# taki0112/vit-tensorflow

Hardware: AMD Instinct MI355X
Metric: images/sec (fwd+bwd) ViT-B/16 224px bf16 (higher is better)
Workload: dtype bf16; 1 GPU; vit_b16_224 fwd+bwd, batch 256/GPU, N(0,1) NHWC images resident in HBM, random-init weights, softmax-CE cotangent, dropout 0; global_batch=256, parallelism=dp1, compute=bf16

## Files before the change

vit-tensorflow_amd/csrc/env.hip:

```cpp
#include "env.h"

#include <cstdio>
#include <cstdlib>
#include <cstring>
#include <mutex>
#include <set>
#include <string>

namespace {

const VitxEnvSwitch kSwitches[] = {
    {"VITX_GENERIC_GEMM", VITX_ENV_PATH, "1: every Dense on the k-ordered fp32-FMA kernel instead of the MFMA kernels"},
    {"VITX_GENERIC_ATTN", VITX_ENV_PATH, "1: materialised attention (batched products + row softmax) instead of the fused kernel"},
    {"VITX_DEEPVIT_FUSED", VITX_ENV_PATH, "0: DeepViT Re-attention forward as batched GEMMs + head-axis kernels instead of the one-kernel form"},
    {"VITX_DEEPVIT_FUSED_BWD", VITX_ENV_PATH, "0: DeepViT Re-attention backward as batched GEMMs + point / row kernels"},
    {"VITX_CAIT_FUSED", VITX_ENV_PATH, "0: CaiT talking-heads forward as batched GEMMs + chain kernel instead of the one-kernel form"},
    {"VITX_CAIT_QKV_CAT", VITX_ENV_PATH, "0: CaiT patch stage: to_q and to_kv as two Dense launches each way (rounds d(y1) twice)"},
    {"VITX_LN_SCALE_FUSED", VITX_ENV_PATH, "0: CaiT LayerScale VJP as a pass of its own instead of on the LayerNorm VJP (bias gradient from the bf16 rounding)"},
    {"VITX_CHAIN_MFMA", VITX_ENV_PATH, "0: talking-heads chain kernels with in-lane FMAs instead of the fp32 matrix pipe"},
    {"VITX_UNFUSED_HEADOPS", VITX_ENV_PATH, "1: head-axis operations (mix / softmax / LayerNorm over heads) as one kernel each"},
    {"VITX_WGRAD_TRANSPOSE", VITX_ENV_PATH, "1: weight gradients through explicit bf16 transposes + the NT kernel"},
    {"VITX_GELU_TABLE", VITX_ENV_PATH, "0: fc1 epilogue evaluates the degree-7 polynomial GELU instead of the LDS table (another rounding of gelu, both inside a bf16 ulp)"},
    {"VITX_LAST_BLOCK_FULL", VITX_ENV_PATH, "1: the last block of a cls-pooled bf16 ViT on every token row instead of the class rows only (same logits; eight of its parameter gradients sum in another order); read per forward"},
    {"VITX_X3_ATTN", VITX_ENV_PATH, "BF16X3 handles: 1 fused split-operand attention (default), 2 materialised scores + split-operand products, 0 exact fp32 products"},
    {"VITX_F32_MFMA", VITX_ENV_TUNING, "0: parity-mode GEMMs on the scalar-FMA kernel instead of the fp32 matrix pipe (same bits)"},
    {"VITX_GEMM_KERNEL", VITX_ENV_TUNING, "force one NT tile variant (1, 2, 3, 5, 6, 7, 9, 10, 11, 13; +256 direct / +512 LDS-staged epilogue); every variant adds in the same K order"},
    {"VITX_GEMM_TAIL_KERNEL", VITX_ENV_TUNING, "with VITX_GEMM_KERNEL=13 / 11: tile variant (1, 3, 10) of the tail launch (tail balancing)"},
    {"VITX_GEMM_TAIL", VITX_ENV_TUNING, "1: the per-shape measurement also times the tail-balanced forms (off by default: loses inside the step)"},
    {"VITX_GEMM_AUTOTUNE", VITX_ENV_TUNING, "0: static variant rule instead of the first-launch measurement"},
    {"VITX_GEMM_AUTOTUNE_LOG", VITX_ENV_TUNING, "1: print the measured variant choices"},
    {"VITX_GEMM_WALK", VITX_ENV_TUNING, "0: no XCD-owned row bands in the persistent NT kernel"},
    {"VITX_GEMM_GRID", VITX_ENV_TUNING, "n: persistent workgroups per launch (default 256)"},
    {"VITX_GEMM_PHASE", VITX_ENV_TUNING, "n: start-phase offsets between the persistent workgroups of an XCD (sleeps only)"},
    {"VITX_EPI_WIDE", VITX_ENV_TUNING, "0: 4-B instead of 16-B-per-lane epilogue accesses"},
    {"VITX_NT", VITX_ENV_TUNING, "bits: non-temporal stores (1 = gelu' of the fc1 epilogue, 16 = d(y) of the fc1 / qkv input gradients; default 17)"},
    {"VITX_REVERSE", VITX_ENV_TUNING, "bits: row tiles walked back to front for operands larger than the memory-side cache (1 forward, 2 input gradients)"},
    {"VITX_REVERSE_MIN_MB", VITX_ENV_TUNING, "operand size from which VITX_REVERSE applies"},
    {"VITX_MLP_BWD_ORDER", VITX_ENV_TUNING, "0: fc2 weight gradient between the producer and the consumers of d(hpre)"},
    {"VITX_BGEMM_PAIRS", VITX_ENV_TUNING, "0: the batched products of the materialised attention backward as four launches instead of two (same bits)"},
    {"VITX_ATTN_BWD_SPLIT", VITX_ENV_TUNING, "1: fused attention backward as two launches (same bits)"},
    {"VITX_GLP_SKIP", VITX_ENV_TUNING, "0: LayerNorm VJPs always write the bf16 copy of the residual gradient"},
    {"VITX_SCORE_BF16", VITX_ENV_TUNING, "0: DeepViT / CaiT score tensors that only batched products read stay fp32 planes (same bits)"},
    {"VITX_LN_CORESIDENT", VITX_ENV_TUNING, "1: LayerNorm VJP of 768-wide bf16 rows as 4-wave, 96-register blocks that fit beside a resident weight-gradient GEMM (experiment; partials summed in another order)"},
    {"VITX_LN_CO_BLOCKS", VITX_ENV_TUNING, "blocks of the co-resident LayerNorm VJP form (default 1024; 256 = one 4-wave block per CU, what fits beside a resident GEMM workgroup)"},
    {"VITX_SIDE_STREAM", VITX_ENV_TUNING, "0 one stream; 1 weight gradients on a lowest-priority side stream (default); 2 the same at the highest priority"},
    {"VITX_LN_REDUCE_SIDE_ROWS", VITX_ENV_TUNING, "LayerNorm VJPs of fewer rows keep their small reductions on the main stream (default 8192)"},
    {"VITX_SC_KEEP_MB", VITX_ENV_TUNING, "budget of the score tensors kept per block for the backward; blocks beyond it recompute (same bits)"},
    {"VITX_RECOMPUTE_SCORES", VITX_ENV_TUNING, "1: materialised attention recomputes its score tensors in the backward (same bits)"},
    {"VITX_WGRAD_WGS", VITX_ENV_TUNING, "workgroups per weight-gradient launch (default 128 up to 24576 token rows, else 256); changes the split-K slice count: fixed-order sums in another order"},
    {"VITX_SG_BLOCKS", VITX_ENV_TUNING, "blocks per LayerScale-gradient launch"},
    {"VITX_DV_CPI", VITX_ENV_TUNING, "chunks per image of the DeepViT one-kernel forward (tests: the multi-tile loop at small batches)"},
    {"VITX_COMM_PRIORITY", VITX_ENV_TUNING, "priority of the communication stream: 1 highest (default), 0 default, -1 lowest"},
    {"VITX_COMM_TIMING", VITX_ENV_TUNING, "0: no event brackets around the collectives (every Dense launch behind a bucket then takes the one-tile form)"},
    {"VITX_COMM_WAIT_ON_CHAIN", VITX_ENV_TUNING, "1: the compute stream (not the communication stream) waits for the weight-gradient stream's share of a reported range"},
    {"VITX_COMM_STREAM_EARLY", VITX_ENV_TUNING, "0: the communication stream is created at vitx_comm_overlap instead of with the handle's other streams (A/B: it may then share a command-processor pipe with the compute stream)"},
    {"VITX_COMM_SHARED", VITX_ENV_TUNING, "1: the Dense launches behind a bucket take the one-tile-per-workgroup form for as long as its collective was measured to last (default 0: persistent grids throughout, faster with emulated collectives)"},
    {"VITX_RCCL_LIB", VITX_ENV_TUNING, "path of the collective library to dlopen instead of librccl.so (tests/fake_rccl: two ranks on one GPU)"},
    {"VITX_GEMM_STAGGER", VITX_ENV_DIAG, "bits reach the NT kernels' experiment field: 1 no DMA wait, 2 no DMA issue (WRONG GEMM results)"},
    {"VITX_GEMM_XP", VITX_ENV_DIAG, "1: vitx_bench_gemm accepts the NT kernels' experiment bits (results invalid)"},
    {"VITX_TN_XP", VITX_ENV_DIAG, "bits: weight-gradient kernel without DMA wait / DMA issue / fragment reads (WRONG weight gradients)"},
    {"VITX_DV_XP", VITX_ENV_DIAG, "bits: DeepViT one-kernel forward without kept tensors / stage 2 / stage 3 (WRONG results)"},
    {"VITX_DVB_XP", VITX_ENV_DIAG, "bits: DeepViT one-kernel backward without one of its stages (WRONG results)"},
    {"VITX_BENCH_ZERO", VITX_ENV_DIAG, "vitx_bench_gemm on zero operands (DVFS / power-limit experiment)"},
    {"VITX_GEMM_STAMPS", VITX_ENV_DIAG, "vitx_bench_gemm prints the cycle stamps of the tile phases (needs the stamps build of gemm_bf16_pipe.hip)"},
};
constexpr int kNumSwitches = (int)(sizeof(kSwitches) / sizeof(kSwitches[0]));

#ifdef VITX_DIAG
constexpr int kDiagBuild = 1;
#else
constexpr int kDiagBuild = 0;
#endif

}

const VitxEnvSwitch* vitx_env_table(int* n) {
  if (n) *n = kNumSwitches;
  return kSwitches;
}
int vitx_env_diag_build() { return kDiagBuild; }

const char* vitx_env(const char* name) {
  const VitxEnvSwitch* sw = nullptr;
  for (int i = 0; i < kNumSwitches; ++i)
    if (std::strcmp(kSwitches[i].name, name) == 0) { sw = &kSwitches[i]; break; }
  if (!sw) {
    fprintf(stderr, "[vitx] internal error: environment switch %s is not in the registry (csrc/env.hip)\n", name);
    abort();
  }
  const char* v = getenv(name);
  if (v && sw->cls == VITX_ENV_DIAG && !kDiagBuild) {
    static std::mutex mu;
    static std::set<std::string> told;
    std::lock_guard<std::mutex> lk(mu);
    if (told.insert(name).second)
      fprintf(stderr, "[vitx] %s is a diagnostic switch that may corrupt results: ignored by this (release) library; use lib/libvitx_diag.so "
                      "(python vit-tensorflow_amd/build.py --diag)\n", name);
    return nullptr;
  }
  return v;
}
```

vit-tensorflow_amd/csrc/gemm_bf16_tn.hip:

```cpp
#include "gemm_bf16_common.h"

namespace {

__device__ __forceinline__ bf16x8 tr_frag(const char* p0, const char* p1) {
  typedef __attribute__((address_space(3))) s16x4 lds_s16x4;
  const s16x4 lo = __builtin_amdgcn_ds_read_tr16_b64_v4i16((lds_s16x4*)p0);
  const s16x4 hi = __builtin_amdgcn_ds_read_tr16_b64_v4i16((lds_s16x4*)p1);
  union { struct { s16x4 a, b; } s; bf16x8 v; } u;
  u.s.a = lo; u.s.b = hi;
  return u.v;
}

template <int BT, int WM, int WN, int MODE>
__global__ __launch_bounds__(WM * WN * 64) void gemm_bf16_tn_kernel(Bf16GemmArgs g, EpiParams ep, int tiles_m, int tiles_n,
                                                                    int kt_per_split) {
  constexpr int NW = WM * WN;
  constexpr int WTM = BT / WM, WTN = BT / WN;
  constexpr int MT = WTM / 32, NT = WTN / 32;
  constexpr int ROWB = BT * 2;
  constexpr int LPR = ROWB / 16;
  constexpr int RPI = 64 / LPR;
  constexpr int OP_BYTES = BK * ROWB, STAGE = 2 * OP_BYTES;
  constexpr int INSTR = BK / RPI / NW;
  static_assert(BK % (RPI * NW) == 0, "token rows must split evenly over the waves");
  extern __shared__ __attribute__((aligned(16))) char smem[];

  const int nwg = gridDim.x, bid = blockIdx.x;
  const int xcd = bid & 7, q8 = nwg >> 3, r8 = nwg & 7;
  const int work = (xcd < r8 ? xcd * (q8 + 1) : r8 * (q8 + 1) + (xcd - r8) * q8) + (bid >> 3);
  const int tiles = tiles_m * tiles_n;
  const int z = work / tiles;
  const int logical = work - z * tiles;
  const int tile_m = logical / tiles_n, tile_n = logical - tile_m * tiles_n;
  const int nk_total = g.K / BK;
  const int kt0 = z * kt_per_split;
  const int nk = min(kt_per_split, nk_total - kt0);

  const int tid = threadIdx.x, lane = tid & 63;
  const int wave = __builtin_amdgcn_readfirstlane(tid >> 6);
  const int wm = wave / WN, wn = wave - wm * WN;

  const bf16_t* Ag = g.A + (int64_t)kt0 * BK * g.lda + (int64_t)tile_m * BT;
  const bf16_t* Bg = g.B + (int64_t)kt0 * BK * g.ldb + (int64_t)tile_n * BT;
  uint32_t offA[INSTR], offB[INSTR];
#pragma unroll
  for (int i = 0; i < INSTR; ++i) {
    const int row = (wave * INSTR + i) * RPI + lane / LPR;
    const int pc = lane % LPR;
    const int c = ((((pc >> 1) ^ (2 * (row & 3))) << 1) | (pc & 1));
    offA[i] = (uint32_t)(row * (int)g.lda + c * 8) * 2u - (uint32_t)((i & 3) * 1024);
    offB[i] = (uint32_t)(row * (int)g.ldb + c * 8) * 2u - (uint32_t)((i & 3) * 1024);
  }
  constexpr int P = 2 * INSTR;
  constexpr int Q = MT * NT;
  constexpr int N3 = (P + 2) / 3, N0 = (P + 1) / 3, N1 = P - N3 - N0;
  const i32x4 rsA = vitx_make_rsrc(Ag), rsB = vitx_make_rsrc(Bg);
  const uint32_t lds_w = vitx_lds_addr(smem) + (uint32_t)wave * (INSTR * 1024u);
  const uint32_t a_kstep = (uint32_t)(BK * g.lda * 2), b_kstep = (uint32_t)(BK * g.ldb * 2);
  auto issue_piece = [&](int buf, int kt, auto p_c) {
    constexpr int p = decltype(p_c)::value;
    const uint32_t base = lds_w + (uint32_t)buf * STAGE;
    if constexpr (p < INSTR) {
      if constexpr ((p & 3) == 0) vitx_dma16(rsA, base + p * 1024, offA[p], (uint32_t)kt * a_kstep);
      else vitx_dma16_cont<(p & 3) * 1024>(rsA, offA[p], (uint32_t)kt * a_kstep);
    } else {
      constexpr int q = p - INSTR;
      if constexpr ((q & 3) == 0) vitx_dma16(rsB, base + OP_BYTES + q * 1024, offB[q], (uint32_t)kt * b_kstep);
      else vitx_dma16_cont<(q & 3) * 1024>(rsB, offB[q], (uint32_t)kt * b_kstep);
    }
  };
  auto stage = [&](int buf, int kt) { static_for<P>([&](auto p_c) { issue_piece(buf, kt, p_c); }); };

  f32x16 acc[MT][NT];
#pragma unroll
  for (int i = 0; i < MT; ++i)
#pragma unroll
    for (int j = 0; j < NT; ++j)
#pragma unroll
      for (int r = 0; r < 16; ++r) acc[i][j][r] = 0.f;

  const int q = lane & 15, G = lane >> 4, khalf = lane >> 5;
  const int trow = q >> 2;
  const int piece = (G & 1) * 32 + (q & 3) * 8;
  auto row_addr = [&](int m, int feat_byte) {
    const int gran = (feat_byte >> 5) ^ (2 * (m & 3));
    return m * ROWB + (gran << 5) + (feat_byte & 31);
  };
  bf16x8 fa[2][MT], fb[2][NT];
  auto load_frags = [&](bf16x8(&af)[MT], bf16x8(&bfr)[NT], const char* base, int ks) {
    const int m0 = 16 * ks + 8 * khalf + trow, m1 = m0 + 4;
#pragma unroll
    for (int i = 0; i < MT; ++i) {
      const int fbyte = (wm * WTM + i * 32) * 2 + piece;
      af[i] = tr_frag(base + row_addr(m0, fbyte), base + row_addr(m1, fbyte));
    }
#pragma unroll
    for (int j = 0; j < NT; ++j) {
      const int fbyte = (wn * WTN + j * 32) * 2 + piece;
      bfr[j] = tr_frag(base + OP_BYTES + row_addr(m0, fbyte), base + OP_BYTES + row_addr(m1, fbyte));
    }
  };
  auto mfma_range = [&](auto cur_c, auto first_c, auto last_c) {
    constexpr int CUR = decltype(cur_c)::value, FIRST = decltype(first_c)::value, LAST = decltype(last_c)::value;
    static_for<(LAST > FIRST ? LAST - FIRST : 0)>([&](auto d) {
      constexpr int idx = FIRST + decltype(d)::value, i = idx / NT, j = idx % NT;
      acc[i][j] = __builtin_amdgcn_mfma_f32_32x32x16_bf16(fb[CUR][j], fa[CUR][i], acc[i][j], 0, 0, 0);
    });
  };
  const int xp = g.stagger;
  auto handover = [&]() {
    if (xp & 1) asm volatile("s_waitcnt lgkmcnt(0)" ::: "memory");
    else asm volatile("s_waitcnt vmcnt(0) lgkmcnt(0)" ::: "memory");
    __builtin_amdgcn_s_barrier();
    asm volatile("" ::: "memory");
  };

  if (nk > 0) stage(0, 0);
  if (nk > 1) stage(1, 1);
  handover();
  load_frags(fa[0], fb[0], smem, 0);
  bool pending = false;
  constexpr int QH = Q < 2 ? Q : 2;
  for (int kt = 0; kt < nk; ++kt) {
    const char* base = smem + (kt & 1) * STAGE;
    static_for<BK / 16>([&](auto ks_c) {
      constexpr int ks = decltype(ks_c)::value, CUR = ks & 1;
      constexpr int NP = ks == 3 ? N3 : (ks == 0 ? N0 : (ks == 1 ? N1 : 0));
      constexpr int FP = ks == 3 ? 0 : (ks == 0 ? N3 : N3 + N0);
      if constexpr (ks + 1 < BK / 16) {
        mfma_range(ic<CUR>{}, ic<0>{}, ic<QH>{});
        __builtin_amdgcn_sched_barrier(0);
        if (!(xp & 4)) load_frags(fa[CUR ^ 1], fb[CUR ^ 1], base, ks + 1);
      } else {
        handover();
        mfma_range(ic<CUR>{}, ic<0>{}, ic<QH>{});
        __builtin_amdgcn_sched_barrier(0);
        if (!(xp & 4)) load_frags(fa[0], fb[0], smem + ((kt + 1) & 1) * STAGE, 0);
        pending = kt + 2 < nk && !(xp & 2);
      }
      __builtin_amdgcn_sched_barrier(0);
      if constexpr (NP > 0) {
        const int ikt = ks == 3 ? kt + 2 : kt + 1;
        const int ibuf = ikt & 1;
        static_for<NP>([&](auto d_c) {
          constexpr int d = decltype(d_c)::value;
          mfma_range(ic<CUR>{}, ic<(QH + d < Q ? QH + d : Q)>{}, ic<(QH + 1 + d < Q ? QH + 1 + d : Q)>{});
          if (pending) issue_piece(ibuf, ikt, ic<FP + d>{});
          __builtin_amdgcn_sched_barrier(0);
        });
        mfma_range(ic<CUR>{}, ic<(QH + NP < Q ? QH + NP : Q)>{}, ic<Q>{});
        if constexpr (FP + NP == P) pending = false;
      } else {
        mfma_range(ic<CUR>{}, ic<QH>{}, ic<Q>{});
      }
      __builtin_amdgcn_sched_barrier(0);
    });
  }

  const int64_t out_off = (int64_t)z * ep.partial_stride;
  const bool interior = epilogue_fast_ok(ep, MODE) && (tile_m + 1) * BT <= ep.M && (tile_n + 1) * BT <= ep.N;
  const float4 z4 = make_float4(0.f, 0.f, 0.f, 0.f);
#pragma unroll
  for (int i = 0; i < MT; ++i) {
    const int row = tile_m * BT + wm * WTM + i * 32 + (lane & 31);
#pragma unroll
    for (int j = 0; j < NT; ++j) {
      const int col0 = tile_n * BT + wn * WTN + j * 32 + 4 * khalf;
#pragma unroll
      for (int qq = 0; qq < 4; ++qq) {
        const float4 v = make_float4(acc[i][j][4 * qq], acc[i][j][4 * qq + 1], acc[i][j][4 * qq + 2], acc[i][j][4 * qq + 3]);
        if (interior) epilogue_fast4<MODE, bf16_t, false, false>(ep, row, col0 + 8 * qq, v, z4, z4, z4, out_off);
        else epilogue_apply4<MODE, bf16_t>(ep, row, col0 + 8 * qq, v, out_off);
      }
    }
  }
}

template <int BT, int WM, int WN>
void launch_tn_variant(const Bf16GemmArgs& g, const EpiParams& ep, hipStream_t s) {
  constexpr int SMEM = 2 * 2 * BK * BT * 2;
  auto kern = gemm_bf16_tn_kernel<BT, WM, WN, EPI_PARTIAL>;
  vitx_set_max_smem((const void*)kern, SMEM);
  const int tiles_m = (int)ceil_div(g.M, BT), tiles_n = (int)ceil_div(g.N, BT);
  const int nk = g.K / BK;
  const int split = g.split_k > 1 ? g.split_k : 1;
  const int per = (int)ceil_div(nk, split);
  const int zs = (int)ceil_div(nk, per);
  dim3 grid((unsigned)(tiles_m * tiles_n * zs)), block(WM * WN * 64);
  hipLaunchKernelGGL(kern, grid, block, SMEM, s, g, ep, tiles_m, tiles_n, per);
}

}

int gemm_bf16_tn_tile(int kernel, int M, int N) { kernel &= 15; return (kernel == 1 || (M <= 128 && N <= 128)) ? 128 : 256; }
void launch_gemm_bf16_tn(const Bf16GemmArgs& g0, const EpiParams& ep, hipStream_t s) {
  static const int xp = [] {
    const char* v = vitx_env("VITX_TN_XP");
    const int x = v ? atoi(v) : 0;
    if (x) fprintf(stderr, "[vitx] VITX_TN_XP=%d: timing experiment -- weight gradients are WRONG in this process\n", x);
    return x;
  }();
  Bf16GemmArgs g = g0;
  g.stagger = xp;
  {
    const int nk = g.K / BK, split = g.split_k > 1 ? g.split_k : 1;
    const int64_t slice_rows = ceil_div(nk, split) * BK;
    if ((slice_rows * std::max(g.lda, g.ldb) + 256) * 2 >= (1LL << 31)) {
      fprintf(stderr, "[vitx] launch_gemm_bf16_tn: a K slice of %lld rows x %lld features exceeds the 2 GiB buffer range -- NOT launched; use more slices\n",
              (long long)slice_rows, (long long)std::max(g.lda, g.ldb));
      return;
    }
  }
  if (gemm_bf16_tn_tile(g.kernel, g.M, g.N) == 128) launch_tn_variant<128, 2, 2>(g, ep, s);
  else launch_tn_variant<256, 2, 4>(g, ep, s);
}
```

vit-tensorflow_amd/csrc/kernels.h:

```cpp
#pragma once
#include "common.h"
#include "epilogue.h"

struct GenericGemmArgs {
  const void* A = nullptr;
  const void* B = nullptr;
  int M = 0, N = 0, K = 0;
  int64_t sam = 0, sak = 1, sbk = 0, sbn = 1;
  int nb = 1, nh = 1;
  int64_t sAb = 0, sAh = 0, sBb = 0, sBh = 0;
  int k_last = 0;
  int x3 = 0;
};
void launch_gemm_generic(const GenericGemmArgs& g, const EpiParams& ep, int mode, int ta, int tb, int to, hipStream_t s);
bool gemm_f32_mfma_supported(const GenericGemmArgs& g, int ta, int tb, int to);
void launch_gemm_f32_mfma(const GenericGemmArgs& g, const EpiParams& ep, int mode, hipStream_t s);
void gemm_f32_mfma_read_env();
bool gemm_bf16x3_supported(const GenericGemmArgs& g, int ta, int tb, int to);
void launch_gemm_bf16x3(const GenericGemmArgs& g, const EpiParams& ep, int mode, hipStream_t s);

bool headchain_supported(int h, int nk);
int64_t headchain_ws_elems(int h);
void launch_cait_chain_fwd(const float* s0, const float* wpre, const float* wpost, float* a1_or_null, float* a2, int b, int h, int nq, int nk,
                           int64_t ld, hipStream_t s);
void launch_cait_chain_bwd(const float* s0, const float* a1, float* da_inout, const float* wpre, const float* wpost, float* ws, float* dwpre,
                           float* dwpost, int b, int h, int nq, int nk, int64_t ld, hipStream_t s, bf16_t* ds_lp = nullptr);
bool cait_chain_bwd_bf16_out_ok();
void launch_deepvit_chain_fwd(float* s0_inout, const float* wre, const float* gamma, const float* beta, float* mixed_or_null, float* a2, int keep,
                              int b, int h, int nq, int nk, int64_t ld, float eps, hipStream_t s);
void launch_deepvit_chain_bwd(const float* a0, const float* mixed, float* da_inout, const float* wre, const float* gamma, float* ws, float* dwre,
                              float* dgamma, float* dbeta, int b, int h, int nq, int nk, int64_t ld, float eps, hipStream_t s);

bool bgemm_mfma_supported(const GenericGemmArgs& g, int ta, int tb, int to, int mode);
void launch_bgemm_mfma(const GenericGemmArgs& g, const EpiParams& ep, int ta, int to, hipStream_t s);
void launch_bgemm_mfma_pair(const GenericGemmArgs& g1, const EpiParams& ep1, int ta1, int to1, const GenericGemmArgs& g2, const EpiParams& ep2, int ta2,
                            int to2, hipStream_t s);

struct Bf16GemmArgs {
  const bf16_t* A = nullptr;
  const bf16_t* B = nullptr;
  int64_t lda = 0, ldb = 0;
  int M = 0, N = 0, K = 0;
  int split_k = 1;
  int kernel = 0;
  unsigned long long* stamps = nullptr;
  int phase = 0;
  int reverse_m = 0;
  int shared_gpu = 0;
  int walk = 0;
  int stagger = 0;
  int tail = 0;
};
void launch_gemm_bf16(const Bf16GemmArgs& g, const EpiParams& ep, int mode, hipStream_t s);
int gemm_bf16_variant_for(int mode, int M, int N, int K, int has_scale, int shared_gpu);
bool gemm_bf16_gelu_table_active();
int gemm_bf16_tile_m(int kernel, int M, int N);
int gemm_bf16_tile_n(int kernel, int M, int N);
int gemm_bf16_num_slices(int K, int split_k);
void gemm_bf16_set_shared_gpu(int on);
void gemm_bf16_allow_320(int on);
void launch_gemm_bf16_tn(const Bf16GemmArgs& g, const EpiParams& ep, hipStream_t s);
int gemm_bf16_tn_tile(int kernel, int M, int N);

bool attn_bf16_supported(int n, int dim_head);
void launch_attn_bf16_fwd(const bf16_t* qkv, bf16_t* o, float* lse, int b, int n, int h, float scale, const bf16_t* zero_page, int reverse,
                          hipStream_t s, int nq_live = 0);
bool attn_x3_supported(int n, int dim_head);
void launch_attn_x3_fwd(const float* qkv, float* o, float* lse, int b, int n, int h, float scale, hipStream_t s);
void launch_attn_x3_bwd(const float* qkv, const float* o, const float* d_o, const float* lse, float* dqkv, int b, int n, int h, float scale, hipStream_t s);
void launch_attn_bf16_bwd(const bf16_t* qkv, const bf16_t* o, const bf16_t* d_o, const float* lse, float* dsum_ws,
                          bf16_t* dqkv, int b, int n, int h, float scale, const bf16_t* zero_page, hipStream_t s, int nq_live = 0);

constexpr int ATTN_STREAM_MAX_N = 1 << 20;
bool attn_stream_supported(int n, int dim_head);
bool attn_stream_fits(int b, int n, int h);
void launch_attn_stream_fwd(const bf16_t* qkv, bf16_t* o, float* lse, int b, int n, int h, float scale, hipStream_t s);
void launch_attn_stream_bwd(const bf16_t* qkv, const bf16_t* o, const bf16_t* d_o, const float* lse, float* dsum_ws, bf16_t* dqkv, int b, int n, int h,
                            float scale, hipStream_t s);

constexpr int LSA_N_MAX = 288;
bool attn_lsa_supported(int n, int dim_head);
int64_t attn_lsa_ws_elems(int b, int n, int h);
void launch_attn_lsa_fwd(const void* qkv, void* o, float* lse, int is_bf16, int b, int n, int h, int dim_head, const float* temperature, hipStream_t s);
void launch_attn_lsa_bwd(const void* qkv, const void* o, const void* d_o, const float* lse, float* dsum_ws, void* dqkv, int is_bf16, int b, int n, int h,
                         int dim_head, const float* temperature, float* dtemperature, float* part_ws, hipStream_t s);
bool attn_small_supported(int n, int dim_head);
void launch_attn_small_fwd(const void* qkv, void* o, float* lse, int is_bf16, int b, int n, int h, int dim_head, float scale, hipStream_t s,
                           const float* bias = nullptr);
void launch_attn_small_bwd(const void* qkv, const void* o, const void* d_o, const float* lse, float* dsum_ws, void* dqkv, int is_bf16, int b, int n, int h,
                           int dim_head, float scale, hipStream_t s, const float* bias = nullptr);
bool attn_window_supported(int n, int dim_head);
void launch_attn_window_fwd(const bf16_t* qkv, bf16_t* o, float* lse, const float* bias, int b, int n, int h, float scale, hipStream_t s);
void launch_attn_window_bwd(const bf16_t* qkv, const bf16_t* o, const bf16_t* d_o, const float* lse, bf16_t* dqkv, const float* bias, int b, int n, int h,
                            float scale, hipStream_t s);
void launch_cf_to_dilated(const float* x, float* tokens, int b, int H, int W, int g, int c, hipStream_t s);
void launch_cf_from_dilated(const float* tokens, float* x, int b, int H, int W, int g, int c, hipStream_t s);
struct CfDpbParams { const float* t[14]; };
int64_t cf_dpb_ws_elems(int wsz);
void launch_cf_dpb_bias(const CfDpbParams& p, int d4, int wsz, float* ws, float* bias, hipStream_t s);
void launch_cf_cols_put(const float* src, float* dst, int64_t rows, int w, int ld, int col0, hipStream_t s);
void launch_cf_cols_get(const float* src, float* dst, int64_t rows, int w, int ld, int col0, hipStream_t s);

void launch_spt_fwd(const float* img, void* rows, int rows_bf16, int64_t ldo, float* mean, float* rstd, const float* gamma, const float* beta, int b,
                    int H, int W, int C, int p, float eps, hipStream_t s);
int64_t spt_bwd_ws_elems(int feat);
void launch_spt_bwd(const float* img, float* d_rows, int64_t ld, const float* mean, const float* rstd, const float* gamma, float* ws, float* dgamma,
                    float* dbeta, int want_dx, int b, int H, int W, int C, int p, hipStream_t s);
void launch_spt_dimg(const float* dx, int64_t ld, float* dimg, int b, int H, int W, int C, int p, hipStream_t s);

void launch_cct_im2col(const float* x, float* rows, int b, int H, int W, int C, int k, int st, int Kp, hipStream_t s);
void launch_cct_relu_maxpool_fwd(const float* conv, float* out, int b, int H, int W, int C, int k, int st, hipStream_t s);
void launch_cct_relu_maxpool_bwd(const float* conv, const float* dout, float* dconv, int b, int H, int W, int C, int k, int st, hipStream_t s);

void launch_nest_to_blocks(const float* x, const float* pos, float* tokens, int b, int nb, int hb, int wb, int c, hipStream_t s, int nbx = 0);
void launch_nest_from_blocks(const float* tokens, float* x, int b, int nb, int hb, int wb, int c, hipStream_t s, int nbx = 0);
void launch_nest_dpos(const float* dtokens, float* part, float* dpos, int nseq, int n, int c, hipStream_t s);
void launch_nest_maxpool_fwd(const float* x, float* out, int b, int H, int W, int C, int k, int st, hipStream_t s);
void launch_nest_maxpool_bwd(const float* x, const float* dout, float* dx, int b, int H, int W, int C, int k, int st, hipStream_t s);

bool attn_fewkey_supported(int nq, int nk, int dim_head);
void launch_attn_fewkey_fwd(const bf16_t* q, const bf16_t* kv, bf16_t* o, float* lse, int b, int nq, int nk, int heads, int64_t ldq, int64_t ldkv,
                            int64_t ldo, float scale, hipStream_t s);
void launch_attn_fewkey_bwd(const bf16_t* q, const bf16_t* kv, const bf16_t* o, const bf16_t* d_o, const float* lse, bf16_t* dq, bf16_t* dkv, int b, int nq,
                            int nk, int heads, int64_t ldq, int64_t ldkv, int64_t ldo, int64_t lddo, int64_t lddq, int64_t lddkv, float scale, hipStream_t s);

constexpr int MANYKEY_MAX = 320;
bool attn_manykey_supported(int nq, int nk, int dim_head);
void launch_attn_manykey_fwd(const bf16_t* q, const bf16_t* kv, bf16_t* o, float* lse, int b, int nq, int nk, int heads, int64_t ldq, int64_t ldkv,
                             int64_t ldo, float scale, hipStream_t s);
void launch_attn_manykey_bwd(const bf16_t* q, const bf16_t* kv, const bf16_t* o, const bf16_t* d_o, const float* lse, bf16_t* dq, bf16_t* dkv, int b, int nq,
                             int nk, int heads, int64_t ldq, int64_t ldkv, int64_t ldo, int64_t lddo, int64_t lddq, int64_t lddkv, float scale, hipStream_t s);

void launch_twins_patch_gather(const float* x, float* out, int b, int H, int W, int C, int p, int64_t ld, hipStream_t s);
void launch_twins_patch_scatter(const float* dpatches, int64_t ld, float* dx, int b, int H, int W, int C, int p, hipStream_t s);
void launch_twins_kunfold(const void* x, void* out, int is_bf16, int b, int H, int W, int C, int k, int64_t ldo, hipStream_t s);
void launch_twins_kfold_add(const void* dwin, int64_t ld, void* dx, int is_bf16, int b, int H, int W, int C, int k, hipStream_t s);
void launch_twins_peg_fwd(const float* x, const float* kern, const float* bias, float* out, int b, int H, int W, int C, int kp, hipStream_t s);
void launch_twins_peg_bwd_dx(const float* dy, const float* kern, float* dx, int b, int H, int W, int C, int kp, hipStream_t s);
int64_t twins_peg_ws_elems(int C, int kp);
void launch_twins_peg_bwd_dkern(const float* x, const float* dy, float* ws, float* dkern, int b, int H, int W, int C, int kp, hipStream_t s);

int64_t cvt_dwbn_ws_elems(int C, int k);
void launch_cvt_dwbn_fwd(const void* x, int is_bf16, const float* kern, const float* gamma, const float* beta, const float* mov_mean, const float* mov_var,
                         int training, float eps, float* conv, double* stats, void* y, int64_t ldy, float* ws, int b, int H, int W, int C, int k, int st,
                         hipStream_t s);
void launch_cvt_bn_bwd(const void* dy, int is_bf16, int64_t lddy, const float* conv, const double* stats, const float* gamma, float* dgamma, float* dbeta,
                       float* dconv, float* ws, int64_t rows, int C, hipStream_t s);
void launch_cvt_dw_bwd_dkern(const void* x, int is_bf16, const float* dconv, float* ws, float* dkern, int b, int H, int W, int C, int k, int st, hipStream_t s);
void launch_cvt_dw_bwd_dx(const float* dconv_q, const float* kern_q, const float* dconv_kv, const float* kern_kv, int st_kv, void* dx, int is_bf16, int b, int H,
                          int W, int C, int k, hipStream_t s);

void launch_unfold(const float* img, void* out, int out_bf16, int b, int H, int W, int C, int ph, int pw,
                   int64_t ldo, hipStream_t s);
void launch_fold_add(const float* dpatches, int64_t ld, float* dimg, int b, int H, int W, int C, int ph, int pw, hipStream_t s);
void extract_patches_geometry(int H, int W, int k, int st, int* oh, int* ow, int* pad_top, int* pad_left);
void launch_extract_patches(const float* x, float* out, int b, int H, int W, int C, int k, int st, hipStream_t s);
void launch_extract_patches_bwd(const float* dout, float* dx, int b, int H, int W, int C, int k, int st, hipStream_t s);
void launch_cls_pos_row(float* x, const float* cls, const float* pos, int b, int ntok, int d, int64_t ldx, hipStream_t s);
void launch_layernorm_fwd(const float* x, int64_t ldx, const float* gamma, const float* beta, void* y, int y_bf16,
                          int64_t ldy, float* mean, float* rstd, int rows, int d, float eps, hipStream_t s);
void launch_layernorm_bwd(const void* dy, int dy_bf16, int64_t lddy, const float* x, int64_t ldx, const float* mean,
                          const float* rstd, const float* gamma, const float* g_in, int64_t ldgi, float* g_out, int64_t ldgo,
                          void* g_lp, int64_t ldglp, float* partial_ws, float* dgamma, float* dbeta, float* gsum, int rows, int d,
                          hipStream_t s, int* deferred = nullptr);
void launch_layernorm_bwd_reduce(float* partial_ws, int nparts, int d, float* dgamma, float* dbeta, float* gsum, hipStream_t s);
int64_t layernorm_bwd_ws_elems(int d);
bool layernorm_bwd_scale_ok(int d);
void launch_layernorm_bwd_scale(const bf16_t* dy, int64_t lddy, const float* x, int64_t ldx, const float* mean, const float* rstd, const float* gamma,
                                const float* g_in, int64_t ldgi, float* g_out, int64_t ldgo, bf16_t* dbr, int64_t lddbr, const bf16_t* nf, int64_t ldnf,
                                const float* nscale, float* partial_ws, int rows, int d, hipStream_t s, int* nparts);
void launch_layernorm_bwd_scale_reduce(float* partial_ws, int nparts, int d, float* dgamma, float* dbeta, float* dscale, float* dbias, const float* nscale,
                                       hipStream_t s);
void launch_colsum(const void* x, int is_bf16, int64_t ld, int rows, int cols, float* partial_ws, float* out, hipStream_t s);
int64_t colsum_ws_elems(int cols);
void launch_reduce_partials(const float* partial, int nparts, int64_t stride, int64_t n, float* out, float alpha, hipStream_t s);
void launch_reduce_partials3(const float* partial, int nparts, int64_t stride, int64_t seg, int nseg, float* out0, float* out1, float* out2,
                             float* ws2, float alpha, hipStream_t s);
void launch_convert_weight(const float* w, int in, int out, bf16_t* wn, int64_t ldwn, bf16_t* wt, int64_t ldwt, hipStream_t s);
struct ConvertDesc { const float* w; bf16_t* wn; bf16_t* wt; int64_t ldwn, ldwt; int in, out, tiles_x, block0; };
void launch_convert_weights_batched(const ConvertDesc* descs_dev, int n, int total_blocks, hipStream_t s);
void launch_transpose_bf16(const bf16_t* in, int64_t ldi, int rows, int cols, bf16_t* out, int64_t ldo, hipStream_t s);
void launch_convert(const float* in, int64_t ldi, void* out, int out_bf16, int64_t ldo, int rows, int cols, int64_t out_cols_zero_to,
                    hipStream_t s);
void launch_to_f32(const void* in, int in_bf16, int64_t ldi, float* out, int64_t ldo, int rows, int cols, hipStream_t s);
void launch_set_token_row(float* x, const float* tok, int b, int ntok, int row, int d, hipStream_t s);
void launch_copy_rows(const void* src, int64_t src_stride_bytes, void* dst, int64_t dst_stride_bytes, int rows, int row_bytes, hipStream_t s);
void launch_mean_pool(const float* x, int b, int ntok, int d, float* out, hipStream_t s, int stride_tok = 0);
void launch_mean_pool_bwd(const float* dp, int b, int ntok, int d, float* g, hipStream_t s, int stride_tok = 0);
void launch_batch_reduce(const float* g, int b, int ntok, int d, int j0, int nj, float* out, hipStream_t s);
void launch_extract_rows(const float* g, int b, int ntok, int tok_off, int np, int d, void* out, int out_bf16, int64_t ldo, hipStream_t s);
void launch_sum_rows(const float* in, int rows, int d, float* out, hipStream_t s);
void launch_ce_grad(const float* logits, int64_t ld, const int32_t* labels, int b, int nc, float inv_batch, float* dlogits,
                    float* loss, hipStream_t s);
void launch_adamw(float* p, const float* g, float* m, float* v, int64_t n, float lr, float b1, float b2, float eps, float wd, int step, hipStream_t s);
void launch_sgd(float* p, const float* g, float* m, int64_t n, float lr, float mom, float wd, hipStream_t s);
void launch_fill_zero(void* p, int64_t bytes, hipStream_t s);
void launch_fill_random_bf16(bf16_t* p, int64_t n, uint32_t seed, float scale, hipStream_t s);
void launch_max_rel_diff(const void* a, const void* b, int is_bf16, int64_t rows, int cols, int64_t lda, int64_t ldb, float* out_max, hipStream_t s);
void launch_dropout(void* x, int is_bf16, int64_t n, float rate, uint64_t seed, uint32_t site, hipStream_t s);
void launch_axpy_resid(const float* resid, const float* f, const float* scale, float* out, void* keep, int keep_bf16, int64_t rows, int d,
                       hipStream_t s);
void launch_branch_grad(const float* g, const float* scale, void* out, int out_bf16, int64_t rows, int d, float rate, uint64_t seed,
                        uint32_t site, hipStream_t s);
void launch_resid_add(const float* resid, const void* t, int t_bf16, float* out, int64_t n, hipStream_t s);

void launch_softmax_rows(float* sc, int64_t rows, int n, int64_t ld, hipStream_t s);
void launch_softmax_bwd_rows(const float* p, float* dp_inout, int64_t rows, int n, int64_t ld, hipStream_t s);
int64_t deepvit_point_bwd_ws_elems(int h);
void launch_deepvit_point_bwd(const float* a0, float* da_inout, const float* w, const float* gamma, float* ws, float* dw,
                              float* dgamma, float* dbeta, int b, int h, int nq, int nk, int64_t ld, float eps, hipStream_t s);
bool deepvit_attn_fused_supported(int h, int dim_head, int nq, int nk);
bool cait_attn_fused_supported(int h, int dim_head, int nq, int nk);
void launch_cait_attn_fwd(const bf16_t* q, const bf16_t* k, const bf16_t* v, int64_t ldq, int64_t ldk, int64_t ldv, int64_t qb, int64_t kb, int64_t vb,
                          bf16_t* o, int64_t ldo, int64_t ob, const float* wpre, const float* wpost, float* s0_keep, float* a1_keep, float* a2_keep,
                          int keep, int b, int h, int nq, int nk, int64_t ld, float scale, const bf16_t* zero_page, hipStream_t s);
int64_t deepvit_attn_bwd_ws_elems(int b, int h, int nq);
void launch_deepvit_attn_bwd(const bf16_t* q, const bf16_t* k, const bf16_t* v, int64_t ldq, int64_t ldk, int64_t ldv, int64_t qb, int64_t kb, int64_t vb,
                             const bf16_t* d_o, int64_t ldo, int64_t ob, const float* p_keep, const float* w, const float* gamma, float* ds_out,
                             bf16_t* dq, int64_t lddq, int64_t dqb, float* ws, float* dw, float* dgamma, float* dbeta, int b, int h, int nq, int nk,
                             int64_t ld, float scale, float eps, const bf16_t* zero_page, hipStream_t s, int ds_bf16 = 0);
void launch_deepvit_attn_fwd(const bf16_t* q, const bf16_t* k, const bf16_t* v, int64_t ldq, int64_t ldk, int64_t ldv, int64_t qb,
                             int64_t kb, int64_t vb, bf16_t* o, int64_t ldo, int64_t ob, const float* w, const float* gamma,
                             const float* beta, float* p_keep, float* a2_keep, int keep, int b, int h, int nq,
                             int nk, int64_t ld, float scale, float eps, const bf16_t* zero_page, hipStream_t s);
bool deepvit_point_fwd_supported(int h, int nk);
int64_t deepvit_point_ws_elems(int b, int h, int nq);
void launch_deepvit_point_fwd(float* s0_inout, float* stats_ws, const float* w, const float* gamma, const float* beta, float* mixed, float* a2,
                              int keep, int b, int h, int nq, int nk, int64_t ld, float eps, hipStream_t s);
void launch_headmix_fwd(const float* in, const float* w, float* out, int b, int h, int nq, int nk, int64_t ld, hipStream_t s);
void launch_headmix_bwd(const float* in, const float* dout, const float* w, float* din, float* dw_partial_ws, float* dw,
                        int b, int h, int nq, int nk, int64_t ld, hipStream_t s);
int64_t headmix_ws_elems(int b, int h, int nq, int nk);
void launch_headnorm_fwd(const float* in, const float* gamma, const float* beta, float* out, int b, int h, int nq, int nk,
                         int64_t ld, float eps, hipStream_t s);
void launch_headnorm_bwd(const float* in, const float* dout, const float* gamma, float* din, float* partial_ws, float* dgamma,
                         float* dbeta, int b, int h, int nq, int nk, int64_t ld, float eps, hipStream_t s);
void launch_concat_ctx(const void* y, int y_bf16, const float* context, void* ctx, int ctx_bf16, int b, int nq, int nc, int d,
                       hipStream_t s);
void launch_split_ctx_bwd(const void* dctx, int is_bf16, void* dy, float* dcontext, int b, int nq, int nc, int d, hipStream_t s);
void launch_add_T(void* a_inout, const void* b_in, int is_bf16, int64_t n, hipStream_t s);
void launch_scale_grad(const void* fx, int is_bf16, int64_t ldf, const float* g, int64_t ldg, int rows, int d, float* partial_ws,
                       float* dscale, hipStream_t s, const float* scale_or_null = nullptr, void* out_or_null = nullptr, int64_t ldo = 0,
                       float* dbias_or_null = nullptr);
void launch_mul_scale(const float* g, int64_t ldg, const float* scale, void* out, int out_bf16, int64_t ldo, int rows, int d,
                      hipStream_t s);
void launch_broadcast_rows(const float* src, int d, float* dst, int rows, hipStream_t s);

void launch_index_inverse(const int32_t* idx, int64_t ldi, int b, int j0, int j1, int n, int32_t* inv, hipStream_t s);
void launch_gather_rows(const float* src, int64_t src_batch_stride, const int32_t* idx, int64_t ldi, int j0, int b, int k, int d, float* out,
                        hipStream_t s);
void launch_scatter_rows(const float* src, int k_src, const int32_t* inv, int j0, int j1, int b, int n, int d, float* dst, hipStream_t s);
void launch_table_grad(const float* src, int k_src, const int32_t* inv, int j0, int j1, int b, int n, int d, int accumulate, float* dtab,
                       hipStream_t s);
void launch_mae_assemble(const float* proj, const float* mask_token, const float* dpos, const int32_t* idx, int b, int np, int nm, int d, float* out,
                         hipStream_t s);
void launch_select_rowsum(const float* x, const int32_t* inv_or_null, int j0, int j1, int b, int n, int d, float* partial_ws, float* out,
                          hipStream_t s);
void launch_simmim_select(float* x, const int32_t* inv, const float* mask_token, const float* pos, int b, int n, int d, hipStream_t s);
void launch_zero_selected_rows(float* x, const int32_t* inv, int64_t rows, int d, hipStream_t s);
void launch_scatter_by_index(const float* src, const int32_t* idx, int b, int k, int d, float* dst, int64_t dst_batch_stride, int row0, hipStream_t s);
void launch_mpp_labels(const float* img, int b, int H, int W, int C, int p, int bits, float mpv, int has_norm, const float* mean, const float* std_,
                       const int32_t* idx, int k, int32_t* labels, hipStream_t s);
int64_t recon_loss_ws_elems(int64_t count);
void launch_recon_loss(const float* pred, const float* target_or_null, int64_t count, int kind, float scale, float* dpred, float* partial_ws,
                       float* loss_out, hipStream_t s);
```

Before: 7654 images/sec.

## Add 16x16x32 MFMA body to weight-gradient TN kernel for 768-row shapes

Adds a second compute body to the bf16 weight-gradient (TN) GEMM kernel. It uses 16x16x32 MFMA instructions with transposed LDS reads (ds_read_tr16), a matching swizzle, and double-buffered fragment prefetch interleaved with the DMA issue. The 16-wide body is selected by default for 256-tiles with M=768 and N of 768 or 3072, which are the ViT-B qkv/proj/MLP weight-gradient shapes. It can also be forced through an env switch or kernel bits. The goal is better MFMA throughput and scheduling on those shapes, at the cost of a different summation order within a k-step and higher register pressure from the fragment buffers.

Measured after the change: 7679 images/sec (median of 6 runs). Within noise of the previous version (+0.3%).

```diff
diff --git a/vit-tensorflow_amd/csrc/env.hip b/vit-tensorflow_amd/csrc/env.hip
--- a/vit-tensorflow_amd/csrc/env.hip
+++ b/vit-tensorflow_amd/csrc/env.hip
@@ -23,6 +23,7 @@
     {"VITX_GELU_TABLE", VITX_ENV_PATH, "0: fc1 epilogue evaluates the degree-7 polynomial GELU instead of the LDS table (another rounding of gelu, both inside a bf16 ulp)"},
     {"VITX_LAST_BLOCK_FULL", VITX_ENV_PATH, "1: the last block of a cls-pooled bf16 ViT on every token row instead of the class rows only (same logits; eight of its parameter gradients sum in another order); read per forward"},
     {"VITX_X3_ATTN", VITX_ENV_PATH, "BF16X3 handles: 1 fused split-operand attention (default), 2 materialised scores + split-operand products, 0 exact fp32 products"},
+    {"VITX_TN_MFMA", VITX_ENV_PATH, "32 / 16: every weight-gradient launch on the 32x32x16 / 16x16x32 MFMA body instead of the per-tile default (the terms of a k-step add in another order)"},
     {"VITX_F32_MFMA", VITX_ENV_TUNING, "0: parity-mode GEMMs on the scalar-FMA kernel instead of the fp32 matrix pipe (same bits)"},
     {"VITX_GEMM_KERNEL", VITX_ENV_TUNING, "force one NT tile variant (1, 2, 3, 5, 6, 7, 9, 10, 11, 13; +256 direct / +512 LDS-staged epilogue); every variant adds in the same K order"},
     {"VITX_GEMM_TAIL_KERNEL", VITX_ENV_TUNING, "with VITX_GEMM_KERNEL=13 / 11: tile variant (1, 3, 10) of the tail launch (tail balancing)"},
diff --git a/vit-tensorflow_amd/csrc/gemm_bf16_tn.hip b/vit-tensorflow_amd/csrc/gemm_bf16_tn.hip
--- a/vit-tensorflow_amd/csrc/gemm_bf16_tn.hip
+++ b/vit-tensorflow_amd/csrc/gemm_bf16_tn.hip
@@ -11,12 +11,12 @@
   return u.v;
 }
 
-template <int BT, int WM, int WN, int MODE>
+template <int BT, int WM, int WN, int MODE, int MS>
 __global__ __launch_bounds__(WM * WN * 64) void gemm_bf16_tn_kernel(Bf16GemmArgs g, EpiParams ep, int tiles_m, int tiles_n,
                                                                     int kt_per_split) {
   constexpr int NW = WM * WN;
   constexpr int WTM = BT / WM, WTN = BT / WN;
-  constexpr int MT = WTM / 32, NT = WTN / 32;
+  constexpr int MT = WTM / MS, NT = WTN / MS;
   constexpr int ROWB = BT * 2;
   constexpr int LPR = ROWB / 16;
   constexpr int RPI = 64 / LPR;
@@ -40,6 +40,7 @@
   const int wave = __builtin_amdgcn_readfirstlane(tid >> 6);
   const int wm = wave / WN, wn = wave - wm * WN;
 
+  auto swz = [](int m) { return MS == 32 ? 2 * (m & 3) : ((2 * (m & 3)) | ((m >> 3) & 1)); };
   const bf16_t* Ag = g.A + (int64_t)kt0 * BK * g.lda + (int64_t)tile_m * BT;
   const bf16_t* Bg = g.B + (int64_t)kt0 * BK * g.ldb + (int64_t)tile_n * BT;
   uint32_t offA[INSTR], offB[INSTR];
@@ -47,7 +48,7 @@
   for (int i = 0; i < INSTR; ++i) {
     const int row = (wave * INSTR + i) * RPI + lane / LPR;
     const int pc = lane % LPR;
-    const int c = ((((pc >> 1) ^ (2 * (row & 3))) << 1) | (pc & 1));
+    const int c = ((((pc >> 1) ^ swz(row)) << 1) | (pc & 1));
     offA[i] = (uint32_t)(row * (int)g.lda + c * 8) * 2u - (uint32_t)((i & 3) * 1024);
     offB[i] = (uint32_t)(row * (int)g.ldb + c * 8) * 2u - (uint32_t)((i & 3) * 1024);
   }
@@ -71,6 +72,7 @@
   };
   auto stage = [&](int buf, int kt) { static_for<P>([&](auto p_c) { issue_piece(buf, kt, p_c); }); };
 
+  if constexpr (MS == 32) {
   f32x16 acc[MT][NT];
 #pragma unroll
   for (int i = 0; i < MT; ++i)
@@ -174,12 +176,123 @@
       }
     }
   }
-}
-
-template <int BT, int WM, int WN>
+  } else {
+  f32x4 acc[MT][NT];
+#pragma unroll
+  for (int i = 0; i < MT; ++i)
+#pragma unroll
+    for (int j = 0; j < NT; ++j)
+#pragma unroll
+      for (int r = 0; r < 4; ++r) acc[i][j][r] = 0.f;
+
+  typedef __attribute__((address_space(3))) s16x4 lds_s16x4;
+  const int q = lane & 15, grp = lane >> 4;
+  const int m0 = 8 * grp + (q >> 2);
+  const int lane_off = m0 * ROWB + (q & 3) * 8, key = swz(m0);
+  auto frag_off = [&](int feat) { return lane_off + ((((feat * 2) >> 5) ^ key) << 5); };
+  constexpr int DB = 2, IP = MT - DB;
+  static_assert(IP > 0, "the wave tile needs more than DB rows");
+  s16x4 fa[IP][2], fad[2][DB][2], fb[2][NT][2];
+  auto load_a = [&](auto i_c, const char* kbase) {
+    constexpr int i = decltype(i_c)::value;
+    const char* p = kbase + frag_off(wm * WTM + i * 16);
+    fa[i][0] = __builtin_amdgcn_ds_read_tr16_b64_v4i16((lds_s16x4*)p);
+    fa[i][1] = __builtin_amdgcn_ds_read_tr16_b64_v4i16((lds_s16x4*)(p + 4 * ROWB));
+  };
+  constexpr int XR = 2 * NT + 2 * DB;
+  auto load_x = [&](auto buf_c, auto x_c, const char* kbase) {
+    constexpr int buf = decltype(buf_c)::value, x = decltype(x_c)::value;
+    if constexpr (x < 2 * NT) {
+      const char* p = kbase + OP_BYTES + frag_off(wn * WTN + (x >> 1) * 16) + (x & 1) * 4 * ROWB;
+      fb[buf][x >> 1][x & 1] = __builtin_amdgcn_ds_read_tr16_b64_v4i16((lds_s16x4*)p);
+    } else {
+      constexpr int y = x - 2 * NT;
+      const char* p = kbase + frag_off(wm * WTM + (IP + (y >> 1)) * 16) + (y & 1) * 4 * ROWB;
+      fad[buf][y >> 1][y & 1] = __builtin_amdgcn_ds_read_tr16_b64_v4i16((lds_s16x4*)p);
+    }
+  };
+  auto frag = [](const s16x4(&h)[2]) {
+    union { struct { s16x4 a, b; } s; bf16x8 v; } u;
+    u.s.a = h[0]; u.s.b = h[1];
+    return u.v;
+  };
+  constexpr int N1 = (3 * P + 3) / 4, N0 = P - N1;
+  constexpr int R0 = MT >= 2 ? MT / 2 : 1;
+  const int xp = g.stagger;
+  auto handover = [&]() {
+    if (xp & 1) asm volatile("s_waitcnt lgkmcnt(0)" ::: "memory");
+    else asm volatile("s_waitcnt vmcnt(0) lgkmcnt(0)" ::: "memory");
+    __builtin_amdgcn_s_barrier();
+    asm volatile("" ::: "memory");
+  };
+
+  if (nk > 0) stage(0, 0);
+  if (nk > 1) stage(1, 1);
+  handover();
+  static_for<IP>([&](auto i_c) { load_a(i_c, smem); });
+  static_for<XR>([&](auto x_c) { load_x(ic<0>{}, x_c, smem); });
+  bool pending = false;
+  for (int kt = 0; kt < nk; ++kt) {
+    const char* base = smem + (kt & 1) * STAGE;
+    static_for<2>([&](auto ks_c) {
+      constexpr int ks = decltype(ks_c)::value;
+      constexpr int NP = ks == 1 ? N1 : N0, FP = ks == 1 ? 0 : N1, ROWS = ks == 1 ? MT : R0;
+      if constexpr (ks == 1) {
+        handover();
+        pending = kt + 2 < nk && !(xp & 2);
+      }
+      const char* nbase = ks == 0 ? base + 32 * ROWB : smem + ((kt + 1) & 1) * STAGE;
+      const int ikt = ks == 1 ? kt + 2 : kt + 1;
+      static_for<MT>([&](auto i_c) {
+        constexpr int i = decltype(i_c)::value;
+        static_for<NT>([&](auto j_c) {
+          constexpr int j = decltype(j_c)::value;
+          if constexpr (i < IP) acc[i][j] = __builtin_amdgcn_mfma_f32_16x16x32_bf16(frag(fb[ks][j]), frag(fa[i]), acc[i][j], 0, 0, 0);
+          else acc[i][j] = __builtin_amdgcn_mfma_f32_16x16x32_bf16(frag(fb[ks][j]), frag(fad[ks][i - IP]), acc[i][j], 0, 0, 0);
+        });
+        __builtin_amdgcn_sched_barrier(0);
+        if constexpr (i < IP) {
+          if (!(xp & 4)) {
+            load_a(i_c, nbase);
+            constexpr int X0 = i * XR / IP, X1 = (i + 1) * XR / IP;
+            static_for<X1 - X0>([&](auto d_c) { load_x(ic<(ks ^ 1)>{}, ic<X0 + decltype(d_c)::value>{}, nbase); });
+          }
+        }
+        if constexpr (i < ROWS) {
+          constexpr int D0 = FP + i * NP / ROWS, D1 = FP + (i + 1) * NP / ROWS;
+          if constexpr (D1 > D0)
+            if (pending) static_for<D1 - D0>([&](auto d_c) { issue_piece(ikt & 1, ikt, ic<D0 + decltype(d_c)::value>{}); });
+        }
+        __builtin_amdgcn_sched_barrier(0);
+      });
+    });
+  }
+
+  const int64_t out_off = (int64_t)z * ep.partial_stride;
+  const bool interior = epilogue_fast_ok(ep, MODE) && (tile_m + 1) * BT <= ep.M && (tile_n + 1) * BT <= ep.N;
+  const float4 z4 = make_float4(0.f, 0.f, 0.f, 0.f);
+  const int row0 = tile_m * BT + wm * WTM + q, col00 = tile_n * BT + wn * WTN + 4 * grp;
+  if (interior) {
+#pragma unroll
+    for (int i = 0; i < MT; ++i)
+#pragma unroll
+      for (int j = 0; j < NT; ++j)
+        epilogue_fast4<MODE, bf16_t, false, false>(ep, row0 + i * 16, col00 + j * 16, make_float4(acc[i][j][0], acc[i][j][1], acc[i][j][2], acc[i][j][3]),
+                                                   z4, z4, z4, out_off);
+  } else {
+#pragma unroll
+    for (int i = 0; i < MT; ++i)
+#pragma unroll
+      for (int j = 0; j < NT; ++j)
+        epilogue_apply4<MODE, bf16_t>(ep, row0 + i * 16, col00 + j * 16, make_float4(acc[i][j][0], acc[i][j][1], acc[i][j][2], acc[i][j][3]), out_off);
+  }
+  }
+}
+
+template <int BT, int WM, int WN, int MS>
 void launch_tn_variant(const Bf16GemmArgs& g, const EpiParams& ep, hipStream_t s) {
   constexpr int SMEM = 2 * 2 * BK * BT * 2;
-  auto kern = gemm_bf16_tn_kernel<BT, WM, WN, EPI_PARTIAL>;
+  auto kern = gemm_bf16_tn_kernel<BT, WM, WN, EPI_PARTIAL, MS>;
   vitx_set_max_smem((const void*)kern, SMEM);
   const int tiles_m = (int)ceil_div(g.M, BT), tiles_n = (int)ceil_div(g.N, BT);
   const int nk = g.K / BK;
@@ -193,6 +306,19 @@
 }
 
 int gemm_bf16_tn_tile(int kernel, int M, int N) { kernel &= 15; return (kernel == 1 || (M <= 128 && N <= 128)) ? 128 : 256; }
+int gemm_bf16_tn_mfma_shape(int kernel, int tile, int M, int N) {
+  static const int forced = [] {
+    const char* v = vitx_env("VITX_TN_MFMA");
+    const int x = v ? atoi(v) : 0;
+    return x == 16 || x == 32 ? x : 0;
+  }();
+  const int sel = (kernel >> 16) & 3;
+  if (sel == 1) return 32;
+  if (sel == 2) return 16;
+  if (forced) return forced;
+  if (tile == 256 && M == 768 && (N == 768 || N == 3072)) return 16;
+  return 32;
+}
 void launch_gemm_bf16_tn(const Bf16GemmArgs& g0, const EpiParams& ep, hipStream_t s) {
   static const int xp = [] {
     const char* v = vitx_env("VITX_TN_XP");
@@ -211,6 +337,13 @@
       return;
     }
   }
-  if (gemm_bf16_tn_tile(g.kernel, g.M, g.N) == 128) launch_tn_variant<128, 2, 2>(g, ep, s);
-  else launch_tn_variant<256, 2, 4>(g, ep, s);
-}
+  const int tile = gemm_bf16_tn_tile(g.kernel, g.M, g.N);
+  const int ms = gemm_bf16_tn_mfma_shape(g.kernel, tile, g.M, g.N);
+  if (tile == 128) {
+    if (ms == 16) launch_tn_variant<128, 2, 2, 16>(g, ep, s);
+    else launch_tn_variant<128, 2, 2, 32>(g, ep, s);
+  } else {
+    if (ms == 16) launch_tn_variant<256, 2, 4, 16>(g, ep, s);
+    else launch_tn_variant<256, 2, 4, 32>(g, ep, s);
+  }
+}
diff --git a/vit-tensorflow_amd/csrc/kernels.h b/vit-tensorflow_amd/csrc/kernels.h
--- a/vit-tensorflow_amd/csrc/kernels.h
+++ b/vit-tensorflow_amd/csrc/kernels.h
@@ -61,6 +61,7 @@
 void gemm_bf16_allow_320(int on);
 void launch_gemm_bf16_tn(const Bf16GemmArgs& g, const EpiParams& ep, hipStream_t s);
 int gemm_bf16_tn_tile(int kernel, int M, int N);
+int gemm_bf16_tn_mfma_shape(int kernel, int tile, int M, int N);
 
 bool attn_bf16_supported(int n, int dim_head);
 void launch_attn_bf16_fwd(const bf16_t* qkv, bf16_t* o, float* lse, int b, int n, int h, float scale, const bf16_t* zero_page, int reverse,
```
